# TigreGotico/phoonnx

Hardware: AMD Instinct MI355X
Metric: audio samples/sec (22.05 kHz), batch-32 256-phoneme utterances (higher is better)
Workload: dtype f32 (f16x3 split: fp32 operands as two fp16 planes, three MFMA products, fp32 accumulate)

## Files before the change

phoonnx_amd/build.py:

```python
import os
import shutil
import subprocess
import sys

HERE = os.path.dirname(os.path.abspath(__file__))
CSRC = os.path.join(HERE, "csrc")
LIB = os.path.join(HERE, "libvitsmi.so")
SOURCES = ["vitsmi.hip", "tu_conv_f32.hip", "tu_sx.hip", "tu_sx_s16.hip", "tu_sx_s16p.hip", "tu_sx_s32.hip", "tu_sx_bf16.hip", "tu_sx_h1.hip", "tu_pair.hip", "tu_pair16.hip", "g2p.hip",
           "model.cpp", "onnx_reader.cpp"]
HEADERS = sorted(f for f in os.listdir(CSRC) if f.endswith(".hpp")) + ["../../include/vitsmi.h", "../../include/g2pmi.h"]


def hipcc():
    for c in (os.environ.get("HIPCC"), shutil.which("hipcc"), "/opt/rocm/bin/hipcc"):
        if c and os.path.exists(c):
            return c
    raise RuntimeError("hipcc not found (ROCm toolchain required to build libvitsmi.so)")


def source_sha():
    import hashlib
    h = hashlib.sha256()
    for f in SOURCES + HEADERS:
        h.update(f.encode() + b"\0")
# ... 306 lines not shown
    objdir = os.path.join(HERE, "build")
    os.makedirs(objdir, exist_ok=True)
    base = [hipcc(), "--offload-arch=gfx950", "-O3", "-std=c++17", "-fPIC", "-Wno-unused-result",
            "-Rpass-analysis=kernel-resource-usage"]
    base[1:1] = os.environ.get("VITSMI_CXXFLAGS", "").split()

    isas = {}

    def compile_one(src):
        stem = os.path.splitext(src)[0]
        obj = os.path.join(objdir, stem + ".o")
        if not src.endswith(".hip"):
            r = subprocess.run(base + ["-x", "hip", "-c", os.path.join(CSRC, src), "-o", obj], capture_output=True, text=True)
            return src, obj, r
        tdir = os.path.join(objdir, "temps_" + stem)
        shutil.rmtree(tdir, ignore_errors=True)
        os.makedirs(tdir)
        tobj = os.path.join(tdir, stem + ".o")
        r = subprocess.run(base + ["-save-temps=obj", "-x", "hip", "-c", os.path.join(CSRC, src), "-o", tobj], capture_output=True, text=True)
        if r.returncode == 0:
            os.replace(tobj, obj)
            with open(os.path.join(tdir, stem + "-hip-amdgcn-amd-amdhsa-gfx950.s")) as f:
                isas[src] = f.read()
        shutil.rmtree(tdir, ignore_errors=True)
        return src, obj, r

    with ThreadPoolExecutor(max_workers=min(len(SOURCES), os.cpu_count() or 4)) as ex:
        results = list(ex.map(compile_one, SOURCES))
    spilled, spilled_src = {}, {}
    for src, _, r in results:
        if r.returncode != 0:
            sys.stderr.write(r.stdout + r.stderr)
            raise RuntimeError(f"hipcc failed compiling {src}")
        if verbose:
            sys.stderr.write(r.stderr)
        for k, v in spilling_kernels(r.stderr).items():
            spilled[k] = v
            spilled_src[k] = src
    no_spill = ("conv_sx_kernel", "conv_sx_pair16", "conv_sx_small_kernel", "attention_relpos16_kernel")
    bad = {k: v for k, v in spilled.items() if any(n in k for n in no_spill)}
    if bad:
        raise RuntimeError("kernels with asynchronous inline-asm loads must not spill registers: " + ", ".join(f"{k} ({v})" for k, v in bad.items()))
    hip_units = [u for u in SOURCES if u.endswith(".hip")]
    missing = [u for u in hip_units if u not in isas]
    if missing:
        raise RuntimeError(f"no device assembly was kept for {missing} (-save-temps=obj): the ISA checks cannot run")
# ... 40 lines not shown
```

phoonnx_amd/csrc/conv_engine.hip.hpp:

```cpp
#pragma once
#include <hip/hip_runtime.h>
#include <stdint.h>

#include <cstdio>

#include "sx_split.hip.hpp"

namespace vitsmi {

typedef float f32x16 __attribute__((ext_vector_type(16)));
typedef float f32x4 __attribute__((ext_vector_type(4)));
typedef float f32x2 __attribute__((ext_vector_type(2)));

enum : int {
    PRO_LRELU = 1,
    PRO_MASK = 2,
    EPI_RELU = 4,
    EPI_MASK = 8,
    EPI_RES = 16,
    EPI_ACC = 32,
    EPI_DIV = 64,
    EPI_COUPLING = 128,
    EPI_WN = 256,
    EPI_WN_FIRST = 512,
// ... 429 lines not shown
                for (int r = 0; r < 16; r++) v[r] = v[r] * mk_sel + ad[n % NB][r];
            } else {
#pragma unroll
                for (int r = 0; r < 16; r++) v[r] *= mk_sel;
            }
            if ((flags & EPI_RES) && (flags & EPI_ACC)) {
                float oo[16];
#pragma unroll
                for (int r = 0; r < 16; r++) oo[r] = orow_m[r] >= 0 ? ob[orow_m[r] + tt] : 0.f;
#pragma unroll
                for (int r = 0; r < 16; r++) v[r] += oo[r];
            }
            if (flags & EPI_DIV) {
#pragma unroll
                for (int r = 0; r < 16; r++) v[r] = v[r] / div;
            }
#pragma unroll
            for (int r = 0; r < 16; r++)
                if (orow_m[r] >= 0) obm[orow_m[r] + tt] = lrelu_f(v[r], oslope);
            if (planes_m) {
#pragma unroll
                for (int q = 0; q < 4; q++) {
                    unsigned wa[2], wb[2];
                    split2h_pair_pk(lrelu_f(v[4 * q], oslope), lrelu_f(v[4 * q + 1], oslope), wa[0], wa[1], pk);
                    split2h_pair_pk(lrelu_f(v[4 * q + 2], oslope), lrelu_f(v[4 * q + 3], oslope), wb[0], wb[1], pk);
                    const int64_t cell = ((int64_t)((mblk0 + m) * 4 + q) * T + t) * 8 + 4 * hi;
                    *reinterpret_cast<u32x2 *>(plb + cell) = u32x2{wa[0], wb[0]};
                    *reinterpret_cast<u32x2 *>(plb + plane_elems + cell) = u32x2{wa[1], wb[1]};
                }
            }
            if (ob2 && !is_wn) {
#pragma unroll
                for (int r = 0; r < 16; r++)
                    if (orow_m[r] >= 0) ob2[orow_m[r] + tt] = lrelu_f(v[r], oslope2);
            }
        }
    }
    if (a.peak) sx_publish_peak(a.peak, (int)(blockIdx.x + blockIdx.y + blockIdx.z), pk);
}

inline int conv_tile_m(int cfg) { return cfg == 2 ? 128 : ((cfg == 1 || cfg == 3) ? 64 : 32); }
inline int conv_tile_n(int cfg) {
    switch (cfg) {
        case 0: return 512;
        case 1: return 256;
        case 2: return 128;
        case 3: return 64;
        case 5: return 64;
// ... 75 lines not shown
```

phoonnx_amd/csrc/conv_sx_engine.hip.hpp:

```cpp
#pragma once
#include <hip/hip_runtime.h>
#include <stdint.h>

#include <cstdio>
#include <cstdlib>
#include <string>
#include <utility>

#include "conv_engine.hip.hpp"

#ifndef SX_CFG0_WIDE
#define SX_CFG0_WIDE 0
#endif
#ifndef SX16_SPREAD
#define SX16_SPREAD 0
#endif
#ifndef SX16_PRIO
#define SX16_PRIO 0
#endif
#ifndef SX16_ABL
#define SX16_ABL 0
#endif
#ifndef SX16_NA_SMALL
#define SX16_NA_SMALL 2
// ... 303 lines not shown
            xroff[it] = xrok[it] ? (uint32_t)(((int64_t)kh * T + t) * 32) : 0u;
        }
    }
    auto xload = [&](int chunk) {
        const float *cbase = xrb + (int64_t)(2 * chunk) * T * 8;
        static_for<NXC>([&](auto I) {
            constexpr int it = decltype(I)::value;
            if (it < nxc) {
                xst[it][0] = global_read128_x<0>(xroff[it], cbase);
                xst[it][1] = global_read128_x<16>(xroff[it], cbase);
            }
        });
    };
    auto xstore = [&](uint32_t xoff) {
        const float isl = a.islope;
        static_for<NXC>([&](auto I) {
            constexpr int it = decltype(I)::value;
            if (it < nxc) {
                int kh, col;
                xcell(it, kh, col);
                if (kh < 2) {
                    float v[8];
#pragma unroll
                    for (int e = 0; e < 8; e++) {
                        const float x = xrok[it] ? __uint_as_float(xst[it][e >> 2][e & 3]) : 0.f;
                        v[e] = fmaxf(x, x * isl);
                    }
                    u32x4 w0, w1, w2;
                    unsigned p0[4], p1[4], p2[4];
#pragma unroll
                    for (int e = 0; e < 4; e++) {
                        if constexpr (F16) split2h_pair_pk(v[2 * e], v[2 * e + 1], p0[e], p1[e], pk);
                        else split3_pair(v[2 * e], v[2 * e + 1], p0[e], p1[e], p2[e]);
                    }
                    w0 = u32x4{p0[0], p0[1], p0[2], p0[3]};
                    w1 = u32x4{p1[0], p1[1], p1[2], p1[3]};
                    const uint32_t ad = lds0 + xoff + (uint32_t)(kh * LW + col) * 16u;
                    const uint32_t pb = (uint32_t)(2 * LW) * 16u;
                    ds_write128(ad, w0);
                    if constexpr (NPL > 1) ds_write128(ad + pb, w1);
                    if constexpr (!F16 && NPL > 2) {
                        w2 = u32x4{p2[0], p2[1], p2[2], p2[3]};
                        ds_write128(ad + 2 * pb, w2);
                    }
                }
            }
        });
    };
    const int nxv = RAWIN ? 2 * nxc : (fastx ? nx_issued : nit);

// ... 606 lines not shown
        co0 = u == 1 ? row0 : (row0 / (32 * u)) * 32;
        t = t0 + (wn * NW + n) * 32 + l31;
    };
    auto cell_at = [&](int co0, int r, int t, int q) -> int64_t {
        return ((int64_t)((co0 >> 3) + q) * Tout + (t * u + r)) * 8 + 4 * hi;
    };
    auto issue_adds = [&](auto R, auto P) {
        constexpr int rr = decltype(R)::value, pp = decltype(P)::value;
        constexpr int m = rr / (NW / 2), n0 = (rr % (NW / 2)) * 2;
#pragma unroll
        for (int j = 0; j < 2; j++) {
            int co0, r, t;
            geom(m, n0 + j, co0, r, t);
            const int tl = t < T ? t : T - 1;
#pragma unroll
            for (int q = 0; q < 4; q++) {
                const int64_t c = cell_at(co0, r, tl, q);
                if (respl) {
                    if (res_epi) {
                        float o4[4];
                        if constexpr (H1) {
                            unact4h(*reinterpret_cast<const u32x2 *>(resplb + c), unsl, o4);
                        } else {
                            float h0[4], h1[4];
                            unact4h(*reinterpret_cast<const u32x2 *>(resplb + c), 1.f, h0);
                            unact4h(*reinterpret_cast<const u32x2 *>(resplb + plane_elems + c), 1.f, h1);
#pragma unroll
                            for (int e = 0; e < 4; e++) {
                                const float v = __builtin_fmaf(h1[e], 1.f / 2048.f, h0[e]);
                                o4[e] = v < 0.f ? v * unsl : v;
                            }
                        }
                        adb[pp][j][q] = f32x4{o4[0], o4[1], o4[2], o4[3]};
                    } else if (has_add)
                        adb[pp][j][q] = *reinterpret_cast<const f32x4 *>(rawb + c);
                } else if (has_add)
                    adb[pp][j][q] = *reinterpret_cast<const f32x4 *>(addp + c);
                if (two_adds) ad2[j][q] = *reinterpret_cast<const f32x4 *>(rawb + c);
            }
        }
    };
    if constexpr (PIPE) issue_adds(std::integral_constant<int, 0>{}, std::integral_constant<int, 0>{});
    static_for<NRND>([&](auto R) {
        constexpr int rr = decltype(R)::value;
        constexpr int m = rr / (NW / 2), n0 = (rr % (NW / 2)) * 2;
        constexpr int pp = PIPE ? (rr & 1) : 0;
        if constexpr (PIPE) {
            if constexpr (rr + 1 < NRND) issue_adds(std::integral_constant<int, rr + 1>{}, std::integral_constant<int, (rr + 1) & 1>{});
        } else
            issue_adds(R, std::integral_constant<int, 0>{});
        int co0m, rm, tm;
        geom(m, n0, co0m, rm, tm);
        const int row0 = mt * BM + (wm * MW + m) * 32;
        f32x4 bq[4];
// ... 18 lines not shown
#pragma unroll
                for (int e = 0; e < 4; e++) {
                    if constexpr (F16) v[e] = __builtin_fmaf(acc[m][n][4 * q + e], wsc, bq[q][e]);
                    else v[e] = acc[m][n][4 * q + e] + bq[q][e];
                }
                if constexpr (PRE) v += pre[rr][j][q];
                if (has_add) v += adb[pp][j][q];
                if (two_adds) v += ad2[j][q];
                if (flags & EPI_DIV) {
#pragma unroll
                    for (int e = 0; e < 4; e++) v[e] = v[e] / rdiv;
                }
                if (flags & SX_HAS_RAW) {
                    f32x4 o = v;
                    if (flags & SX_RAW_ACT) {
#pragma unroll
                        for (int e = 0; e < 4; e++) o[e] = fmaxf(v[e], v[e] * oslope);
                    }
                    *reinterpret_cast<f32x4 *>(rawb + cell) = o;
                }
                if (flags & SX_HAS_PL) {
                    f32x4 o = v;
                    if (flags & SX_PL_ACT) {
#pragma unroll
                        for (int e = 0; e < 4; e++) o[e] = fmaxf(v[e], v[e] * oslope2);
                    }
                    unsigned wa[3], wb[3];
                    if constexpr (H1) {
                        wa[0] = cvt1h_pair_pk(o[0], o[1], pk);
                        wb[0] = cvt1h_pair_pk(o[2], o[3], pk);
                    } else if constexpr (F16) {
                        split2h_pair_pk(o[0], o[1], wa[0], wa[1], pk);
                        split2h_pair_pk(o[2], o[3], wb[0], wb[1], pk);
                    } else {
                        split3_pair(o[0], o[1], wa[0], wa[1], wa[2]);
                        split3_pair(o[2], o[3], wb[0], wb[1], wb[2]);
                    }
#pragma unroll
                    for (int pl = 0; pl < NPL; pl++)
                        *reinterpret_cast<u32x2 *>(plb + pl * plane_elems + cell) = u32x2{wa[pl], wb[pl]};
                }
            }
        }
    });
    if constexpr (F16) {
        if (a.peak) {
            if constexpr (S16) sx_publish_peak_at(a.peak, (int)blockIdx.x, pk, reinterpret_cast<float *>(lds_sx));
            else sx_publish_peak(a.peak, (int)blockIdx.x, pk);
// ... 110 lines not shown
    if (rawin && (cfg == 0 || 2 * a.LW > 768 || !a.xr || (long long)a.T * 64 + 64 >= (1ll << 32))) return hipErrorInvalidValue;
    if (a.oslope == 0.f) a.oslope = 1.f;
    if (a.oslope2 == 0.f) a.oslope2 = 1.f;
    if (a.islope == 0.f) a.islope = 1.f;
    if (a.Cin % 16 || a.Cout % 32 || a.Cr % 32 || a.Cout % BM) return hipErrorInvalidValue;
    a.NT = (a.T + BN - 1) / BN;
    a.MT = a.Cout / BM;
    a.B = B;
    const long long nb = (long long)a.NT * B;
    if (nb == 0) return hipSuccess;
    a.xgs = a.NT >= (2 << sx_xcd_group_shift()) ? sx_xcd_group_shift() : 0;
    const long long per_round = 8ll << a.xgs;
    const long long wgs = (nb + per_round - 1) / per_round * per_round * a.MT;
    if (wgs >= (1ll << 31)) return hipErrorInvalidValue;
    dim3 grid((unsigned)wgs, 1, 1);
    int epi = a.flags & (EPI_RES | EPI_ACC | EPI_DIV);
    if (a.out_raw && !(a.flags & SX_NO_RAW_STORE)) epi |= SX_HAS_RAW | (a.oslope != 1.f ? SX_RAW_ACT : 0);
    if (a.out_pl && !(a.flags & SX_GATE)) epi |= SX_HAS_PL | (a.oslope2 != 1.f ? SX_PL_ACT : 0);
    if (a.bias_b) epi |= SX_HAS_BIASB;
    if (a.res_pl && nprod == 2 && (a.flags & EPI_RES)) {
        if (a.res || rawin || (a.flags & (SX_WN_RMW | SX_GATE))) return hipErrorInvalidValue;
        epi |= SX_RES_PL;
        if (a.res_unslope == 0.f) a.res_unslope = 1.f;
    }
    if (a.flags & SX_WN_RMW) {
        const bool p_acc = (a.flags & EPI_ACC) != 0;
        if (rawin || nprod != 2 || a.ups != 1 || (a.row_split < a.Cout && !a.out_raw2) ||
            (a.row_split && !a.out_raw && (p_acc || !a.out_pl)) || a.row_split % 32 || a.Cout % 32 || a.row_split > a.Cout ||
            a.pl_rows % 32 || a.pl_rows > (a.pl_of2 ? a.Cout - a.row_split : a.row_split) || (a.pl_rows && !a.out_pl) || a.bias_b ||
            (a.flags & SX_GATE) || ((a.flags & SX_PLANAR_COUPLING) && !p_acc) ||
            ((a.flags & EPI_RES) && (!a.res || p_acc)) || ((a.flags & EPI_MASK) && !a.len))
            return hipErrorInvalidValue;
        epi = -2;
    }
    if (a.flags & SX_GATE) {
        if (rawin || (cfg != 1 && cfg != 3) || (nprod != 2 && nprod != 6) || a.ups != 1 || (!a.out_raw && !a.out_pl) || (a.Cr & 63) ||
            lds < (size_t)2 * (sx_tile_n(cfg) / 64) * 4 * 1024)
            return hipErrorInvalidValue;
        epi |= SX_GATE | SX_HAS_RAW;
    }
    const bool early_ok = rawin && (nprod == 2 || (nprod == 6 && cfg == 2)) && (a.flags & EPI_RES) && !(a.flags & (DBG_NO_DMA | DBG_NO_EPI)) &&
                          a.res == a.xr && a.ups == 1 && a.out_raw && !(a.flags & SX_NO_RAW_STORE) && !a.out_pl && !a.bias_b &&
                          a.oslope == 1.f && (!(a.flags & EPI_DIV) || (a.flags & EPI_ACC));
    if (early_ok && epi != -2) epi |= SX_RES_EARLY;
    if (epi != -2) {
        if ((epi & EPI_RES) && !((nprod == 1 || (epi & SX_RES_PL)) ? (const void *)a.res_pl : (const void *)a.res)) return hipErrorInvalidValue;
// ... 187 lines not shown
```

phoonnx_amd/csrc/conv_sx_pair.hip.hpp:

```cpp
#pragma once
#include <cstdlib>
#include "conv_sx_engine.hip.hpp"

namespace vitsmi {

struct SxPairArgs {
    const float *xr;
    float islope, mslope;
    int T;
    const u32x4 *wp1, *wp2;
    const float *bias1, *bias2;
    float wscale1, wscale2;
    float *out_raw;
    const float *zeros;
    int C, nchunks;
    int K1, dil1, pad1;
    int K2, dil2, pad2;
    int LW1;
    unsigned x_bytes;
    int LW2;
    unsigned y_chunk_bytes;
    int BNo, NT, B;
    int flags;
    float div;
// ... 8 lines not shown
    int nchain;
    unsigned a_ring;
    unsigned bias_off;
    unsigned long long *prof;
    SxRagged rag;
    int xgs = 0;
};

#ifndef SX_PAIR_PROF
#define SX_PAIR_PROF 0
#endif
#ifndef SX_PAIR_SHARED_A
#define SX_PAIR_SHARED_A 0
#endif
#ifndef SX_PAIR_ALIAS
#define SX_PAIR_ALIAS 0
#endif
#ifndef SX_PAIR_DEPTH32
#define SX_PAIR_DEPTH32 2
#endif
#ifndef SX_PAIR_DEPTH64
#define SX_PAIR_DEPTH64 2
#endif
#ifndef SX_PAIR_EARLY_ACC
#define SX_PAIR_EARLY_ACC 0
#endif
#ifndef SX_PAIR_WGS32
#define SX_PAIR_WGS32 3
#endif
#ifndef SX_PAIR_EARLY32
#define SX_PAIR_EARLY32 1
#endif
#ifndef SX_PAIR_ST_SC1
#define SX_PAIR_ST_SC1 0
#endif
#ifndef SX_PAIR_ONE_READ64
#define SX_PAIR_ONE_READ64 1
#endif
#ifndef SX_PAIR_ONE_READ32
#define SX_PAIR_ONE_READ32 1
#endif
template <int MW, int NW, int WM, int WN, int EPI, bool CHAIN, int NCH = 1>
__global__ __launch_bounds__(256, (NW == 2 && !SX_PAIR_EARLY_ACC && NCH == 1) ? SX_PAIR_WGS32 : 2) void conv_sx_pair_kernel(SxPairArgs a) {
    constexpr int BN = NW * WN * 32, NH = NW / 2;
    static_assert(NCH == 1 || (CHAIN && NW == 2 && (EPI & EPI_ACC) == 0), "fused chains: 32 channels, no external running sum");
    constexpr bool ONE_READ = NW == 4 ? SX_PAIR_ONE_READ64 != 0 : SX_PAIR_ONE_READ32 != 0;
    constexpr bool EARLY = ONE_READ || (NW == 2 && SX_PAIR_EARLY32);
    constexpr int DEPTH = NW == 2 ? SX_PAIR_DEPTH32 : SX_PAIR_DEPTH64;
    static_assert(DEPTH >= 2 && DEPTH <= 6, "wait_a covers up to five younger sets");
    constexpr bool ACC = (EPI & EPI_ACC) != 0 && SX_PAIR_EARLY_ACC;
    static_assert(!(ONE_READ && ACC), "the running sum is not pulled into the single-read prologue");
    static_assert(WM * WN == 4 && MW == 1 && BN == 256, "one block row per wave, 256 columns");
    constexpr int NPW = 2, STEPBYTES = WM * MW * NPW * 1024;
    constexpr int MAXCH = WM * 2;
    extern __shared__ __attribute__((aligned(16))) unsigned char lds_sx[];
    const int tid = threadIdx.x, lane = tid & 63;
    const int wave = __builtin_amdgcn_readfirstlane(tid >> 6);
    const int wm = wave / WN, wn = wave % WN;
    const int l31 = lane & 31, hi = lane >> 5;
    const int wg_xcd = blockIdx.x & 7, wg_seq = blockIdx.x >> 3;
    const int tile_nb = __builtin_amdgcn_readfirstlane(sx_xcd_tile(wg_seq, wg_xcd, a.xgs));
    if (tile_nb >= a.NT * a.B) return;
    const int b = tile_nb / a.NT, t0 = (tile_nb - b * a.NT) * a.BNo;
    const int t1 = t0 - a.pad2;
    const int T = a.T, LW = a.LW1;
    const int TV = __builtin_amdgcn_readfirstlane(sx_valid_cols(a.rag, b, T));
    if (t0 >= TV) return;
    const uint32_t lds0 = (uint32_t)(uintptr_t)lds_sx;
    const uint32_t XB = a.x_bytes;
    const char *wbase1 = reinterpret_cast<const char *>(a.wp1) + wm * (MW * NPW * 1024);
    const char *wbase2 = reinterpret_cast<const char *>(a.wp2) + wm * (MW * NPW * 1024);
    const float *xrb = a.xr + (int64_t)b * a.C * T;
    float pk = 0.f;

    struct ASet {
        u32x4 fa[2];
    };
    const uint32_t voff0 = (uint32_t)lane * 16u;
    auto load_a = [&](ASet &f, const char *wb, int step) {
        const char *sb = wb + (int64_t)step * STEPBYTES;
        f.fa[0] = global_read128<0>(voff0, sb);
        f.fa[1] = global_read128<1024>(voff0, sb);
    };

    f32x4 pre[NW / 2][2][4], ad[EARLY && ACC ? NW / 2 : 1][2][4];
    auto load_res = [&](const float *base, f32x4 (*dst)[2][4]) {
        static_for<NW / 2>([&](auto R) {
            constexpr int rr = decltype(R)::value;
#pragma unroll
            for (int j = 0; j < 2; j++) {
                const int row0 = wm * 32;
                const int t = t1 + (wn * NW + rr * 2 + j) * 32 + l31;
                const int tl = t < 0 ? 0 : (t < T ? t : T - 1);
#pragma unroll
                for (int q = 0; q < 4; q++) {
                    const float *p = base + ((int64_t)((row0 >> 3) + q) * T + tl) * 8 + 4 * hi;
                    if constexpr (EARLY) dst[rr][j][q] = __builtin_bit_cast(f32x4, global_read128_v<0>(p));
                    else dst[rr][j][q] = *reinterpret_cast<const f32x4 *>(p);
                }
            }
        });
    };
    auto load_pre = [&]() { load_res(xrb, pre); };

#if SX_PAIR_PROF
    auto stamp = [&]() {
        unsigned long long t;
        __builtin_amdgcn_sched_barrier(0);
        asm volatile("s_memtime %0\n\ts_waitcnt lgkmcnt(0)" : "=s"(t)::"memory");
        __builtin_amdgcn_sched_barrier(0);
        return t;
    };
    unsigned long long tp[8];
    tp[0] = stamp();
#endif
    if constexpr (NW == 2 && WM == 1 && NCH == 1 && SX_PAIR_SHARED_A != 0)
        for (int g = 0; g < 3; g++)
            if (g < ((a.nchunks * a.K1) >> 1)) {
                const int sub = wave >> 1, pl = wave & 1;
                lds_dma<16>(wbase1 + (int64_t)(2 * g + sub) * STEPBYTES + pl * 1024 + lane * 16,
                            reinterpret_cast<float *>(lds_sx + a.a_ring + (unsigned)((g * 2 + sub) * 2048 + pl * 1024)));
            }
    constexpr bool BIAS_LDS = NCH == 1;
    if constexpr (BIAS_LDS) {
        if (wave == 0) {
            constexpr int CC = WM * 32;
            const int k = lane - (lane >= CC / 4 ? CC / 4 : 0);
            const float *bp = lane < CC / 4 ? a.bias1 : a.bias2;
            const void *src = (bp && lane < CC / 2) ? static_cast<const void *>(bp + 4 * k) : static_cast<const void *>(a.zeros + 4 * (lane & 31));
            lds_dma<16>(src, reinterpret_cast<float *>(lds_sx + a.bias_off));
        }
    }
    auto bias_from_lds = [&](int conv, f32x4 (&bq)[4]) __attribute__((always_inline)) {
        u32x4 t4[4];
#pragma unroll
        for (int q = 0; q < 4; q++)
            asm volatile("ds_read_b128 %0, %1" : "=v"(t4[q]) : "v"(lds0 + a.bias_off + (uint32_t)(conv * (WM * 32) + wm * 32 + 8 * q + 4 * hi) * 4u) : "memory");
        asm volatile("s_waitcnt lgkmcnt(0)" ::: "memory");
        __builtin_amdgcn_sched_barrier(0);
#pragma unroll
        for (int q = 0; q < 4; q++) bq[q] = __builtin_bit_cast(f32x4, t4[q]);
    };
    constexpr int NXC = 3;
    if constexpr (ONE_READ) {
        constexpr int NXH = MAXCH, NG = 2 * MAXCH;
        const int HW = LW - 256, pad1 = a.pad1;
        const int nhc = HW * NG, nxh = (nhc + 255) >> 8;
        u32x4 hst[NXH][2];
        bool hin[NXH], hok[NXH];
        uint32_t hlds[NXH];
        const float *hp[NXH];
#pragma unroll
        for (int it = 0; it < NXH; it++) {
            const int h = it * 256 + tid;
            hin[it] = h < nhc;
            const int g = hin[it] ? h / HW : 0;
            const int c = hin[it] ? h - g * HW : 0;
            const int col = c < pad1 ? c : c + 256;
            const int t = t1 - pad1 + col;
            hok[it] = hin[it] && t >= 0 && t < TV;
            hp[it] = xrb + (hok[it] ? ((int64_t)g * T + t) * 8 : (int64_t)0);
            hlds[it] = lds0 + (uint32_t)(g >> 1) * XB + (uint32_t)((g & 1) * LW + col) * 16u;
        }
        static_for<NXH>([&](auto I) {
            constexpr int it = decltype(I)::value;
            if (it < nxh) {
                hst[it][0] = global_read128_v<0>(hp[it]);
                hst[it][1] = global_read128_v<16>(hp[it]);
            }
        });
        load_pre();
        const float isl = a.islope;
        static_for<NW>([&](auto N) {
            constexpr int n = decltype(N)::value;
            asm volatile("s_waitcnt vmcnt(%0)" ::"n"(4 * (NW - 1 - n)) : "memory");
            __builtin_amdgcn_sched_barrier(0);
#if SX_PAIR_PROF
            if constexpr (n == 0) tp[1] = stamp();
#endif
            if constexpr (n == 0) {
                static_for<NXH>([&](auto I) {
                    constexpr int it = decltype(I)::value;
                    if (it < nxh && hin[it]) {
                        float v[8];
#pragma unroll
                        for (int e = 0; e < 8; e++) {
                            const float x = hok[it] ? __uint_as_float(hst[it][e >> 2][e & 3]) : 0.f;
                            v[e] = fmaxf(x, x * isl);
                        }
                        unsigned p0[4], p1[4];
#pragma unroll
                        for (int e = 0; e < 4; e++) split2h_pair_pk(v[2 * e], v[2 * e + 1], p0[e], p1[e], pk);
                        ds_write128(hlds[it], u32x4{p0[0], p0[1], p0[2], p0[3]});
                        ds_write128(hlds[it] + (uint32_t)(2 * LW) * 16u, u32x4{p1[0], p1[1], p1[2], p1[3]});
                    }
                });
            }
            const int col = (wn * NW + n) * 32 + l31;
            const int t = t1 + col;
            const bool ok = t >= 0 && t < TV;
#pragma unroll
            for (int q = 0; q < 4; q++) {
                float v[4];
#pragma unroll
                for (int e = 0; e < 4; e++) {
                    const float x = ok ? pre[n / 2][n % 2][q][e] : 0.f;
                    v[e] = fmaxf(x, x * isl);
                }
                unsigned wa[2], wb[2];
                split2h_pair_pk(v[0], v[1], wa[0], wa[1], pk);
                split2h_pair_pk(v[2], v[3], wb[0], wb[1], pk);
                const int g = 4 * wm + q;
                const uint32_t cell = lds0 + (uint32_t)(g >> 1) * XB + (uint32_t)((g & 1) * LW + pad1 + col) * 16u + 8u * hi;
                asm volatile("ds_write_b64 %0, %1" ::"v"(cell), "v"(u32x2{wa[0], wb[0]}) : "memory");
                asm volatile("ds_write_b64 %0, %1" ::"v"(cell + (uint32_t)(2 * LW) * 16u), "v"(u32x2{wa[1], wb[1]}) : "memory");
            }
            asm volatile("" : "+v"(pk));
        });
    } else {
        u32x4 xst[MAXCH][NXC][2];
        const int nxc = (2 * LW + 255) >> 8;
        uint32_t xroff[NXC];
        bool xrok[NXC];
        int xkh[NXC], xcol[NXC];
#pragma unroll
        for (int it = 0; it < NXC; it++) {
            const int i = it * 256 + tid;
            const int kh = (i >= LW ? 1 : 0) + (i >= 2 * LW ? 1 : 0);
            const int col = i - kh * LW;
            const int t = t1 - a.pad1 + col;
            xkh[it] = kh;
            xcol[it] = col;
            xrok[it] = it < nxc && kh < 2 && t >= 0 && t < TV;
            xroff[it] = xrok[it] ? (uint32_t)(((int64_t)kh * T + t) * 32) : 0u;
        }
        static_for<MAXCH>([&](auto CH) {
            constexpr int ch = decltype(CH)::value;
            const float *cbase = xrb + (int64_t)(2 * ch) * T * 8;
            static_for<NXC>([&](auto I) {
                constexpr int it = decltype(I)::value;
                if (it < nxc) {
                    xst[ch][it][0] = global_read128_x<0>(xroff[it], cbase);
                    xst[ch][it][1] = global_read128_x<16>(xroff[it], cbase);
                }
            });
        });
        if constexpr (EARLY) {
            load_pre();
            if constexpr (ACC) {
                load_res(a.out_raw + (int64_t)b * a.C * T, ad);
                asm volatile("s_waitcnt vmcnt(16)" ::: "memory");
            } else
                asm volatile("s_waitcnt vmcnt(8)" ::: "memory");
        } else
            asm volatile("s_waitcnt vmcnt(0)" ::: "memory");
#if SX_PAIR_PROF
        tp[1] = stamp();
#endif
        const float isl = a.islope;
        static_for<MAXCH>([&](auto CH) {
            constexpr int ch = decltype(CH)::value;
            static_for<NXC>([&](auto I) {
                constexpr int it = decltype(I)::value;
                if (it < nxc && xkh[it] < 2) {
                    float v[8];
#pragma unroll
                    for (int e = 0; e < 8; e++) {
                        const float x = xrok[it] ? __uint_as_float(xst[ch][it][e >> 2][e & 3]) : 0.f;
                        v[e] = fmaxf(x, x * isl);
                    }
                    unsigned p0[4], p1[4];
#pragma unroll
                    for (int e = 0; e < 4; e++) split2h_pair_pk(v[2 * e], v[2 * e + 1], p0[e], p1[e], pk);
                    const uint32_t ad = lds0 + (uint32_t)ch * XB + (uint32_t)(xkh[it] * LW + xcol[it]) * 16u;
                    ds_write128(ad, u32x4{p0[0], p0[1], p0[2], p0[3]});
                    ds_write128(ad + (uint32_t)(2 * LW) * 16u, u32x4{p1[0], p1[1], p1[2], p1[3]});
                }
            });
        });
    }

    f32x16 acc[NW];
    auto zero_acc = [&]() {
#pragma unroll
        for (int n = 0; n < NW; n++)
#pragma unroll
            for (int r = 0; r < 16; r++) acc[n][r] = 0.f;
    };
    zero_acc();
    u32x4 fb[NW][2];
    auto load_b_half = [&](auto H, uint32_t rows, uint32_t pstride) {
        constexpr int h = decltype(H)::value;
        static_for<NH>([&](auto N) {
            constexpr int n = h * NH + decltype(N)::value;
            fb[n][0] = ds_read128<n * 512>(rows);
            fb[n][1] = ds_read128<n * 512>(rows + pstride);
        });
    };
    auto mma_half = [&](const ASet &f, auto H) {
        constexpr int h = decltype(H)::value;
#pragma unroll
// ... 156 lines not shown
            step(fa1, fa0, 2 * g + 1, true);
        }
    };

    struct ChainPar {
        const char *wb1, *wb2;
        const float *bias1, *bias2;
        float ws1, ws2;
        int K1, dil1, K2, dil2;
        uint32_t xoff, yoff;
    };
    auto chain_par = [&](int ci) {
        ChainPar c;
        if constexpr (NCH == 1) {
            c = ChainPar{wbase1, wbase2, a.bias1, a.bias2, a.wscale1, a.wscale2, a.K1, a.dil1, a.K2, a.dil2, 0u, 0u};
        } else {
            const auto &h = a.ch[ci];
            c = ChainPar{reinterpret_cast<const char *>(h.wp1) + wm * (MW * NPW * 1024),
                         reinterpret_cast<const char *>(h.wp2) + wm * (MW * NPW * 1024),
                         h.bias1, h.bias2, h.wscale1, h.wscale2, h.K1, h.dil1, h.K2, h.dil2, (uint32_t)h.xoff, (uint32_t)h.yoff};
        }
        return c;
    };
    static_assert(NCH == 1 || EARLY, "fused chains keep x in registers from the prologue on");
    const uint32_t ylds = NCH > 1 ? lds0 + (uint32_t)a.nchunks * XB : lds0;
    f32x4 xkeep[NCH > 1 ? NW / 2 : 1][2][4], tot[NCH > 1 ? NW / 2 : 1][2][4];
#if SX_PAIR_ALIAS
    ASet f1s[DEPTH + 1];
    ASet(&f2s)[DEPTH + 1] = f1s;
#else
    ASet f1s[DEPTH + 1], f2s[DEPTH + 1];
#endif
#pragma unroll 1
    for (int ci = 0; ci < NCH; ci++) {
    const ChainPar cp = chain_par(ci);
    if constexpr (NCH > 1) {
        if (ci > 0) {
#pragma unroll
            for (int rr = 0; rr < NW / 2; rr++)
#pragma unroll
                for (int j = 0; j < 2; j++)
#pragma unroll
                    for (int q = 0; q < 4; q++) pre[rr][j][q] = xkeep[rr][j][q];
            zero_acc();
        }
    }
    if constexpr (!SHA) load_a(f1s[0], cp.wb1, 0);
    if (ci == 0) {
        asm volatile("s_waitcnt lgkmcnt(0)" ::: "memory");
#if SX_PAIR_PROF
        tp[2] = stamp();
#endif
        __builtin_amdgcn_s_barrier();
#if SX_PAIR_PROF
        tp[3] = stamp();
#endif
    }
    __builtin_amdgcn_sched_barrier(0);
    if constexpr (SHA)
        run_conv_sha(f1s[0], f1s[1], cp.wb1, cp.K1, cp.dil1, lds0 + (uint32_t)(hi * LW + wn * (NW * 32) + l31 + (int)cp.xoff) * 16u,
                     XB, (uint32_t)(2 * LW) * 16u);
    else
        run_conv(f1s, cp.wb1, cp.K1, cp.dil1, lds0 + (uint32_t)(hi * LW + wn * (NW * 32) + l31 + (int)cp.xoff) * 16u, XB,
                 (uint32_t)(2 * LW) * 16u);

#if SX_PAIR_PROF
    tp[4] = stamp();
#endif
    if constexpr (CHAIN && !EARLY) load_pre();

    if constexpr (!SHA) load_a(f2s[0], cp.wb2, 0);
    asm volatile("s_waitcnt lgkmcnt(0)" ::: "memory");
    __builtin_amdgcn_s_barrier();
    __builtin_amdgcn_sched_barrier(0);
    if constexpr (SHA) sha_prefetch(cp.wb2, cp.K2);
    {
        const float wsc = cp.ws1, msl = a.mslope;
        const float *biasp = cp.bias1 ? cp.bias1 : a.zeros;
        const int b_on = cp.bias1 ? 1 : 0;
        const uint32_t YC = a.y_chunk_bytes, LW2 = (uint32_t)a.LW2;
        const int row0 = wm * 32;
        f32x4 bq[4];
        if constexpr (BIAS_LDS) bias_from_lds(0, bq);
        else {
#pragma unroll
            for (int q = 0; q < 4; q++) bq[q] = *reinterpret_cast<const f32x4 *>(biasp + (row0 + 8 * q + 4 * hi) * b_on);
        }
#pragma unroll
        for (int n = 0; n < NW; n++) {
            const int col = (wn * NW + n) * 32 + l31;
            const int t = t1 + col;
            const bool live = t >= 0 && t < TV;
#pragma unroll
            for (int q = 0; q < 4; q++) {
                float o[4];
#pragma unroll
                for (int e = 0; e < 4; e++) {
                    float v = __builtin_fmaf(acc[n][4 * q + e], wsc, bq[q][e]);
                    if constexpr (CHAIN) {
                        if constexpr (NCH > 1) {
                            if (ci == 0) xkeep[n / 2][n % 2][q][e] = pre[n / 2][n % 2][q][e];
                        }
                        v += pre[n / 2][n % 2][q][e];
                        pre[n / 2][n % 2][q][e] = v;
                    }
                    o[e] = live ? fmaxf(v, v * msl) : 0.f;
                }
                unsigned wa[2], wb[2];
                split2h_pair_pk(o[0], o[1], wa[0], wa[1], pk);
                split2h_pair_pk(o[2], o[3], wb[0], wb[1], pk);
                const int g = 4 * wm + q;
                const uint32_t cell = ylds + (uint32_t)(g >> 1) * YC + ((uint32_t)(g & 1) * LW2 + (uint32_t)(col + a.pad2)) * 16u + 8u * hi;
                asm volatile("ds_write_b64 %0, %1" ::"v"(cell), "v"(u32x2{wa[0], wb[0]}) : "memory");
                asm volatile("ds_write_b64 %0, %1" ::"v"(cell + 2u * LW2 * 16u), "v"(u32x2{wa[1], wb[1]}) : "memory");
            }
            asm volatile("" : "+v"(pk));
        }
    }
    zero_acc();
    asm volatile("s_waitcnt lgkmcnt(0)" ::: "memory");
    __builtin_amdgcn_s_barrier();
    __builtin_amdgcn_sched_barrier(0);
#if SX_PAIR_PROF
    tp[5] = stamp();
#endif

    if constexpr (SHA)
        run_conv_sha(f2s[0], f2s[1], cp.wb2, cp.K2, cp.dil2, ylds + (uint32_t)(hi * a.LW2 + wn * (NW * 32) + l31 + (int)cp.yoff) * 16u,
                     a.y_chunk_bytes, (uint32_t)(2 * a.LW2) * 16u);
    else
        run_conv(f2s, cp.wb2, cp.K2, cp.dil2, ylds + (uint32_t)(hi * a.LW2 + wn * (NW * 32) + l31 + (int)cp.yoff) * 16u,
                 a.y_chunk_bytes, (uint32_t)(2 * a.LW2) * 16u);
#if SX_PAIR_PROF
    tp[6] = stamp();
#endif
    if constexpr (!CHAIN && !EARLY) load_pre();

    {
        constexpr int flags = EPI;
        float *rawb = a.out_raw + (int64_t)b * a.C * T;
        const float wsc = cp.ws2, rdiv = a.div;
        const float *biasp = cp.bias2 ? cp.bias2 : a.zeros;
        const int b_on = cp.bias2 ? 1 : 0;
        const int row0 = wm * 32;
        f32x4 bq[4];
        if constexpr (BIAS_LDS) bias_from_lds(1, bq);
        else {
#pragma unroll
            for (int q = 0; q < 4; q++) bq[q] = *reinterpret_cast<const f32x4 *>(biasp + (row0 + 8 * q + 4 * hi) * b_on);
        }
        static_for<NW / 2>([&](auto R) {
            constexpr int rr = decltype(R)::value;
            f32x4 adl[2][4];
            if constexpr ((flags & EPI_ACC) != 0 && !(EARLY && ACC)) {
#pragma unroll
                for (int j = 0; j < 2; j++) {
                    const int t = t1 + (wn * NW + rr * 2 + j) * 32 + l31;
                    const int tl = t < 0 ? 0 : (t < T ? t : T - 1);
#pragma unroll
                    for (int q = 0; q < 4; q++)
                        adl[j][q] = *reinterpret_cast<const f32x4 *>(rawb + ((int64_t)((row0 >> 3) + q) * T + tl) * 8 + 4 * hi);
                }
            }
#pragma unroll
            for (int j = 0; j < 2; j++) {
                const int n = rr * 2 + j;
                const int col = (wn * NW + n) * 32 + l31;
                const int t = t1 + col;
                const bool kept = !(col < a.pad2 || col >= a.pad2 + a.BNo || t >= TV);
                if constexpr (NCH == 1) {
                    if (!kept) continue;
                }
#pragma unroll
                for (int q = 0; q < 4; q++) {
                    f32x4 v;
#pragma unroll
                    for (int e = 0; e < 4; e++) v[e] = __builtin_fmaf(acc[n][4 * q + e], wsc, bq[q][e]);
                    v += pre[rr][j][q];
                    if constexpr (NCH > 1) {
                        if (ci > 0) v += tot[rr][j][q];
                        tot[rr][j][q] = v;
                        if (ci < NCH - 1 || !kept) continue;
                    }
                    if constexpr ((flags & EPI_ACC) != 0) {
                        if constexpr (EARLY && ACC) v += ad[rr][j][q];
                        else v += adl[j][q];
                    }
                    if constexpr ((flags & EPI_DIV) != 0) {
#pragma unroll
                        for (int e = 0; e < 4; e++) v[e] = v[e] / rdiv;
                    }
#if SX_PAIR_ST_SC1
                    {
                        float *sp = rawb + ((int64_t)((row0 >> 3) + q) * T + t) * 8 + 4 * hi;
                        const f32x4 sv = v;
                        asm volatile("global_store_dwordx4 %0, %1, off sc1" ::"v"(sp), "v"(sv) : "memory");
                    }
#else
                    *reinterpret_cast<f32x4 *>(rawb + ((int64_t)((row0 >> 3) + q) * T + t) * 8 + 4 * hi) = v;
#endif
                }
            }
        });
    }
    }
#if SX_PAIR_PROF
    asm volatile("s_waitcnt vmcnt(0)" ::: "memory");
    tp[7] = stamp();
    if (a.prof && tid == 0) {
// ... 167 lines not shown
```

phoonnx_amd/csrc/sx_split.hip.hpp:

```cpp
#pragma once
#include <hip/hip_runtime.h>
#include <stdint.h>

#include <atomic>

namespace vitsmi {

typedef float sxf32x2 __attribute__((ext_vector_type(2)));
typedef _Float16 f16x2 __attribute__((ext_vector_type(2)));
typedef unsigned u32x4 __attribute__((ext_vector_type(4)));
typedef unsigned u32x2 __attribute__((ext_vector_type(2)));

constexpr int kSxPeakSlots = 64;
constexpr float kF16Max = 65504.f;

inline thread_local bool g_launch_name_on = false;
inline thread_local char g_launch_name[128];

__device__ __forceinline__ unsigned cvt_pk_f16(float lo, float hi) {
    const sxf32x2 v = {lo, hi};
    return __builtin_bit_cast(unsigned, __builtin_convertvector(v, f16x2));
}
__device__ __forceinline__ void split2h_pair(float x, float y, unsigned &w0, unsigned &w1) {
    x = __builtin_amdgcn_fmed3f(x, -65504.f, 65504.f);
    y = __builtin_amdgcn_fmed3f(y, -65504.f, 65504.f);
    w0 = cvt_pk_f16(x, y);
    const f16x2 h = __builtin_bit_cast(f16x2, w0);
    w1 = cvt_pk_f16((x - (float)h[0]) * 2048.f, (y - (float)h[1]) * 2048.f);
}
__device__ __forceinline__ void split2h_pair_pk(float x, float y, unsigned &w0, unsigned &w1, float &pk) {
    pk = __builtin_fmaxf(pk, __builtin_fmaxf(__builtin_fabsf(x), __builtin_fabsf(y)));
    split2h_pair(x, y, w0, w1);
}
__device__ __forceinline__ unsigned cvt1h_pair_pk(float x, float y, float &pk) {
    pk = __builtin_fmaxf(pk, __builtin_fmaxf(__builtin_fabsf(x), __builtin_fabsf(y)));
    return cvt_pk_f16(__builtin_amdgcn_fmed3f(x, -65504.f, 65504.f), __builtin_amdgcn_fmed3f(y, -65504.f, 65504.f));
}
__device__ __forceinline__ void unact4h(u32x2 w, float unslope, float (&o)[4]) {
    const unsigned wx = w.x, wy = w.y;
    const f16x2 a = __builtin_bit_cast(f16x2, wx), b = __builtin_bit_cast(f16x2, wy);
    const float v[4] = {(float)a[0], (float)a[1], (float)b[0], (float)b[1]};
#pragma unroll
    for (int e = 0; e < 4; e++) o[e] = v[e] < 0.f ? v[e] * unslope : v[e];
}

constexpr int kSxPeakStride = 32;
constexpr int kSxMaxDynLds = 160 * 1024 - 256;
inline hipError_t sx_allow_big_lds(const void *kern, std::atomic<uint64_t> &done) {
    int dev = 0;
    if (hipGetDevice(&dev) != hipSuccess) return hipGetLastError();
    const uint64_t bit = 1ull << (dev & 63);
    if (done.load(std::memory_order_acquire) & bit) return hipSuccess;
    const hipError_t e = hipFuncSetAttribute(kern, hipFuncAttributeMaxDynamicSharedMemorySize, kSxMaxDynLds);
    if (e == hipSuccess) done.fetch_or(bit, std::memory_order_release);
    return e;
}
__device__ __forceinline__ void sx_publish_peak_at(unsigned *slots, int slot_idx, float pk, float *s_pk) {
#pragma unroll
    for (int o = 32; o > 0; o >>= 1) pk = __builtin_fmaxf(pk, __shfl_xor(pk, o, 64));
    __syncthreads();
    if ((threadIdx.x & 63) == 0) s_pk[threadIdx.x >> 6] = pk;
    __syncthreads();
    if (threadIdx.x == 0) {
        pk = __builtin_fmaxf(__builtin_fmaxf(s_pk[0], s_pk[1]), __builtin_fmaxf(s_pk[2], s_pk[3]));
        unsigned *slot = slots + (slot_idx & (kSxPeakSlots - 1)) * kSxPeakStride;
        const unsigned bits = __float_as_uint(pk);
// ... 35 lines not shown
```

Measured before the change: 145.2 million.

## Use packed and mixed-precision ALU ops in split/unsplit and lrelu epilogues; drop legacy pair prologue

Rewrites the fp16 two-plane split to build the residual plane with v_fma_mix instructions, fuses the peak tracking into v_max3, and adds packed-f32 leaky-ReLU, FMA and unsplit helpers used across the sx and pair conv kernels. The pair kernel's non-single-read prologue and early-accumulate variants are removed, and LDS writes now use immediate offsets computed per unrolled column. The aim is fewer VALU instructions in the prologue and epilogue of the conv kernels. The new split rounds slightly differently from the old path, and the unsplit now relies on res_unslope >= 1, which is enforced by a new argument check.

```diff
diff --git a/phoonnx_amd/build.py b/phoonnx_amd/build.py
--- a/phoonnx_amd/build.py
+++ b/phoonnx_amd/build.py
@@ -352,6 +352,11 @@
             os.replace(tobj, obj)
             with open(os.path.join(tdir, stem + "-hip-amdgcn-amd-amdhsa-gfx950.s")) as f:
                 isas[src] = f.read()
+            keep = os.environ.get("VITSMI_KEEP_ISA")
+            if keep:
+                os.makedirs(keep, exist_ok=True)
+                with open(os.path.join(keep, stem + ".s"), "w") as f:
+                    f.write(isas[src])
         shutil.rmtree(tdir, ignore_errors=True)
         return src, obj, r
 
diff --git a/phoonnx_amd/csrc/conv_engine.hip.hpp b/phoonnx_amd/csrc/conv_engine.hip.hpp
--- a/phoonnx_amd/csrc/conv_engine.hip.hpp
+++ b/phoonnx_amd/csrc/conv_engine.hip.hpp
@@ -475,8 +475,8 @@
 #pragma unroll
                 for (int q = 0; q < 4; q++) {
                     unsigned wa[2], wb[2];
-                    split2h_pair_pk(lrelu_f(v[4 * q], oslope), lrelu_f(v[4 * q + 1], oslope), wa[0], wa[1], pk);
-                    split2h_pair_pk(lrelu_f(v[4 * q + 2], oslope), lrelu_f(v[4 * q + 3], oslope), wb[0], wb[1], pk);
+                    split2h_pair_pk_c(lrelu_f(v[4 * q], oslope), lrelu_f(v[4 * q + 1], oslope), wa[0], wa[1], pk);
+                    split2h_pair_pk_c(lrelu_f(v[4 * q + 2], oslope), lrelu_f(v[4 * q + 3], oslope), wb[0], wb[1], pk);
                     const int64_t cell = ((int64_t)((mblk0 + m) * 4 + q) * T + t) * 8 + 4 * hi;
                     *reinterpret_cast<u32x2 *>(plb + cell) = u32x2{wa[0], wb[0]};
                     *reinterpret_cast<u32x2 *>(plb + plane_elems + cell) = u32x2{wa[1], wb[1]};
diff --git a/phoonnx_amd/csrc/conv_sx_engine.hip.hpp b/phoonnx_amd/csrc/conv_sx_engine.hip.hpp
--- a/phoonnx_amd/csrc/conv_sx_engine.hip.hpp
+++ b/phoonnx_amd/csrc/conv_sx_engine.hip.hpp
@@ -349,10 +349,9 @@
                 if (kh < 2) {
                     float v[8];
 #pragma unroll
-                    for (int e = 0; e < 8; e++) {
-                        const float x = xrok[it] ? __uint_as_float(xst[it][e >> 2][e & 3]) : 0.f;
-                        v[e] = fmaxf(x, x * isl);
-                    }
+                    for (int e = 0; e < 8; e++) v[e] = xrok[it] ? __uint_as_float(xst[it][e >> 2][e & 3]) : 0.f;
+#pragma unroll
+                    for (int e = 0; e < 4; e++) lrelu_pair(v[2 * e], v[2 * e + 1], isl);
                     u32x4 w0, w1, w2;
                     unsigned p0[4], p1[4], p2[4];
 #pragma unroll
@@ -1005,14 +1004,8 @@
                         if constexpr (H1) {
                             unact4h(*reinterpret_cast<const u32x2 *>(resplb + c), unsl, o4);
                         } else {
-                            float h0[4], h1[4];
-                            unact4h(*reinterpret_cast<const u32x2 *>(resplb + c), 1.f, h0);
-                            unact4h(*reinterpret_cast<const u32x2 *>(resplb + plane_elems + c), 1.f, h1);
-#pragma unroll
-                            for (int e = 0; e < 4; e++) {
-                                const float v = __builtin_fmaf(h1[e], 1.f / 2048.f, h0[e]);
-                                o4[e] = v < 0.f ? v * unsl : v;
-                            }
+                            unsplit4h(*reinterpret_cast<const u32x2 *>(resplb + c),
+                                      *reinterpret_cast<const u32x2 *>(resplb + plane_elems + c), unsl, o4);
                         }
                         adb[pp][j][q] = f32x4{o4[0], o4[1], o4[2], o4[3]};
                     } else if (has_add)
@@ -1077,8 +1070,15 @@
                 if (flags & SX_HAS_PL) {
                     f32x4 o = v;
                     if (flags & SX_PL_ACT) {
-#pragma unroll
-                        for (int e = 0; e < 4; e++) o[e] = fmaxf(v[e], v[e] * oslope2);
+                        if constexpr (F16 && !H1) {
+                            float l[4] = {v[0], v[1], v[2], v[3]};
+                            lrelu_pair(l[0], l[1], oslope2);
+                            lrelu_pair(l[2], l[3], oslope2);
+                            o = f32x4{l[0], l[1], l[2], l[3]};
+                        } else {
+#pragma unroll
+                            for (int e = 0; e < 4; e++) o[e] = fmaxf(v[e], v[e] * oslope2);
+                        }
                     }
                     unsigned wa[3], wb[3];
                     if constexpr (H1) {
@@ -1235,6 +1235,7 @@
         if (a.res || rawin || (a.flags & (SX_WN_RMW | SX_GATE))) return hipErrorInvalidValue;
         epi |= SX_RES_PL;
         if (a.res_unslope == 0.f) a.res_unslope = 1.f;
+        if (!(a.res_unslope >= 1.f)) return hipErrorInvalidValue;
     }
     if (a.flags & SX_WN_RMW) {
         const bool p_acc = (a.flags & EPI_ACC) != 0;
diff --git a/phoonnx_amd/csrc/conv_sx_pair.hip.hpp b/phoonnx_amd/csrc/conv_sx_pair.hip.hpp
--- a/phoonnx_amd/csrc/conv_sx_pair.hip.hpp
+++ b/phoonnx_amd/csrc/conv_sx_pair.hip.hpp
@@ -54,34 +54,18 @@
 #ifndef SX_PAIR_DEPTH64
 #define SX_PAIR_DEPTH64 2
 #endif
-#ifndef SX_PAIR_EARLY_ACC
-#define SX_PAIR_EARLY_ACC 0
-#endif
 #ifndef SX_PAIR_WGS32
 #define SX_PAIR_WGS32 3
 #endif
-#ifndef SX_PAIR_EARLY32
-#define SX_PAIR_EARLY32 1
-#endif
 #ifndef SX_PAIR_ST_SC1
 #define SX_PAIR_ST_SC1 0
 #endif
-#ifndef SX_PAIR_ONE_READ64
-#define SX_PAIR_ONE_READ64 1
-#endif
-#ifndef SX_PAIR_ONE_READ32
-#define SX_PAIR_ONE_READ32 1
-#endif
 template <int MW, int NW, int WM, int WN, int EPI, bool CHAIN, int NCH = 1>
-__global__ __launch_bounds__(256, (NW == 2 && !SX_PAIR_EARLY_ACC && NCH == 1) ? SX_PAIR_WGS32 : 2) void conv_sx_pair_kernel(SxPairArgs a) {
+__global__ __launch_bounds__(256, (NW == 2 && NCH == 1) ? SX_PAIR_WGS32 : 2) void conv_sx_pair_kernel(SxPairArgs a) {
     constexpr int BN = NW * WN * 32, NH = NW / 2;
     static_assert(NCH == 1 || (CHAIN && NW == 2 && (EPI & EPI_ACC) == 0), "fused chains: 32 channels, no external running sum");
-    constexpr bool ONE_READ = NW == 4 ? SX_PAIR_ONE_READ64 != 0 : SX_PAIR_ONE_READ32 != 0;
-    constexpr bool EARLY = ONE_READ || (NW == 2 && SX_PAIR_EARLY32);
     constexpr int DEPTH = NW == 2 ? SX_PAIR_DEPTH32 : SX_PAIR_DEPTH64;
     static_assert(DEPTH >= 2 && DEPTH <= 6, "wait_a covers up to five younger sets");
-    constexpr bool ACC = (EPI & EPI_ACC) != 0 && SX_PAIR_EARLY_ACC;
-    static_assert(!(ONE_READ && ACC), "the running sum is not pulled into the single-read prologue");
     static_assert(WM * WN == 4 && MW == 1 && BN == 256, "one block row per wave, 256 columns");
     constexpr int NPW = 2, STEPBYTES = WM * MW * NPW * 1024;
     constexpr int MAXCH = WM * 2;
@@ -115,7 +99,7 @@
         f.fa[1] = global_read128<1024>(voff0, sb);
     };
 
-    f32x4 pre[NW / 2][2][4], ad[EARLY && ACC ? NW / 2 : 1][2][4];
+    f32x4 pre[NW / 2][2][4];
     auto load_res = [&](const float *base, f32x4 (*dst)[2][4]) {
         static_for<NW / 2>([&](auto R) {
             constexpr int rr = decltype(R)::value;
@@ -127,8 +111,7 @@
 #pragma unroll
                 for (int q = 0; q < 4; q++) {
                     const float *p = base + ((int64_t)((row0 >> 3) + q) * T + tl) * 8 + 4 * hi;
-                    if constexpr (EARLY) dst[rr][j][q] = __builtin_bit_cast(f32x4, global_read128_v<0>(p));
-                    else dst[rr][j][q] = *reinterpret_cast<const f32x4 *>(p);
+                    dst[rr][j][q] = __builtin_bit_cast(f32x4, global_read128_v<0>(p));
                 }
             }
         });
@@ -173,8 +156,7 @@
 #pragma unroll
         for (int q = 0; q < 4; q++) bq[q] = __builtin_bit_cast(f32x4, t4[q]);
     };
-    constexpr int NXC = 3;
-    if constexpr (ONE_READ) {
+    {
         constexpr int NXH = MAXCH, NG = 2 * MAXCH;
         const int HW = LW - 256, pad1 = a.pad1;
         const int nhc = HW * NG, nxh = (nhc + 255) >> 8;
@@ -216,10 +198,9 @@
                     if (it < nxh && hin[it]) {
                         float v[8];
 #pragma unroll
-                        for (int e = 0; e < 8; e++) {
-                            const float x = hok[it] ? __uint_as_float(hst[it][e >> 2][e & 3]) : 0.f;
-                            v[e] = fmaxf(x, x * isl);
-                        }
+                        for (int e = 0; e < 8; e++) v[e] = hok[it] ? __uint_as_float(hst[it][e >> 2][e & 3]) : 0.f;
+#pragma unroll
+                        for (int e = 0; e < 4; e++) lrelu_pair(v[2 * e], v[2 * e + 1], isl);
                         unsigned p0[4], p1[4];
 #pragma unroll
                         for (int e = 0; e < 4; e++) split2h_pair_pk(v[2 * e], v[2 * e + 1], p0[e], p1[e], pk);
@@ -235,80 +216,18 @@
             for (int q = 0; q < 4; q++) {
                 float v[4];
 #pragma unroll
-                for (int e = 0; e < 4; e++) {
-                    const float x = ok ? pre[n / 2][n % 2][q][e] : 0.f;
-                    v[e] = fmaxf(x, x * isl);
-                }
+                for (int e = 0; e < 4; e++) v[e] = ok ? pre[n / 2][n % 2][q][e] : 0.f;
+                lrelu_pair(v[0], v[1], isl);
+                lrelu_pair(v[2], v[3], isl);
                 unsigned wa[2], wb[2];
                 split2h_pair_pk(v[0], v[1], wa[0], wa[1], pk);
                 split2h_pair_pk(v[2], v[3], wb[0], wb[1], pk);
                 const int g = 4 * wm + q;
-                const uint32_t cell = lds0 + (uint32_t)(g >> 1) * XB + (uint32_t)((g & 1) * LW + pad1 + col) * 16u + 8u * hi;
-                asm volatile("ds_write_b64 %0, %1" ::"v"(cell), "v"(u32x2{wa[0], wb[0]}) : "memory");
-                asm volatile("ds_write_b64 %0, %1" ::"v"(cell + (uint32_t)(2 * LW) * 16u), "v"(u32x2{wa[1], wb[1]}) : "memory");
+                const uint32_t cell = lds0 + (uint32_t)(g >> 1) * XB + (uint32_t)((g & 1) * LW + pad1 + wn * (NW * 32) + l31) * 16u + 8u * hi;
+                asm volatile("ds_write_b64 %0, %1 offset:%2" ::"v"(cell), "v"(u32x2{wa[0], wb[0]}), "n"(n * 512) : "memory");
+                asm volatile("ds_write_b64 %0, %1 offset:%2" ::"v"(cell + (uint32_t)(2 * LW) * 16u), "v"(u32x2{wa[1], wb[1]}), "n"(n * 512) : "memory");
             }
             asm volatile("" : "+v"(pk));
-        });
-    } else {
-        u32x4 xst[MAXCH][NXC][2];
-        const int nxc = (2 * LW + 255) >> 8;
-        uint32_t xroff[NXC];
-        bool xrok[NXC];
-        int xkh[NXC], xcol[NXC];
-#pragma unroll
-        for (int it = 0; it < NXC; it++) {
-            const int i = it * 256 + tid;
-            const int kh = (i >= LW ? 1 : 0) + (i >= 2 * LW ? 1 : 0);
-            const int col = i - kh * LW;
-            const int t = t1 - a.pad1 + col;
-            xkh[it] = kh;
-            xcol[it] = col;
-            xrok[it] = it < nxc && kh < 2 && t >= 0 && t < TV;
-            xroff[it] = xrok[it] ? (uint32_t)(((int64_t)kh * T + t) * 32) : 0u;
-        }
-        static_for<MAXCH>([&](auto CH) {
-            constexpr int ch = decltype(CH)::value;
-            const float *cbase = xrb + (int64_t)(2 * ch) * T * 8;
-            static_for<NXC>([&](auto I) {
-                constexpr int it = decltype(I)::value;
-                if (it < nxc) {
-                    xst[ch][it][0] = global_read128_x<0>(xroff[it], cbase);
-                    xst[ch][it][1] = global_read128_x<16>(xroff[it], cbase);
-                }
-            });
-        });
-        if constexpr (EARLY) {
-            load_pre();
-            if constexpr (ACC) {
-                load_res(a.out_raw + (int64_t)b * a.C * T, ad);
-                asm volatile("s_waitcnt vmcnt(16)" ::: "memory");
-            } else
-                asm volatile("s_waitcnt vmcnt(8)" ::: "memory");
-        } else
-            asm volatile("s_waitcnt vmcnt(0)" ::: "memory");
-#if SX_PAIR_PROF
-        tp[1] = stamp();
-#endif
-        const float isl = a.islope;
-        static_for<MAXCH>([&](auto CH) {
-            constexpr int ch = decltype(CH)::value;
-            static_for<NXC>([&](auto I) {
-                constexpr int it = decltype(I)::value;
-                if (it < nxc && xkh[it] < 2) {
-                    float v[8];
-#pragma unroll
-                    for (int e = 0; e < 8; e++) {
-                        const float x = xrok[it] ? __uint_as_float(xst[ch][it][e >> 2][e & 3]) : 0.f;
-                        v[e] = fmaxf(x, x * isl);
-                    }
-                    unsigned p0[4], p1[4];
-#pragma unroll
-                    for (int e = 0; e < 4; e++) split2h_pair_pk(v[2 * e], v[2 * e + 1], p0[e], p1[e], pk);
-                    const uint32_t ad = lds0 + (uint32_t)ch * XB + (uint32_t)(xkh[it] * LW + xcol[it]) * 16u;
-                    ds_write128(ad, u32x4{p0[0], p0[1], p0[2], p0[3]});
-                    ds_write128(ad + (uint32_t)(2 * LW) * 16u, u32x4{p1[0], p1[1], p1[2], p1[3]});
-                }
-            });
         });
     }
 
@@ -511,7 +430,6 @@
         }
         return c;
     };
-    static_assert(NCH == 1 || EARLY, "fused chains keep x in registers from the prologue on");
     const uint32_t ylds = NCH > 1 ? lds0 + (uint32_t)a.nchunks * XB : lds0;
     f32x4 xkeep[NCH > 1 ? NW / 2 : 1][2][4], tot[NCH > 1 ? NW / 2 : 1][2][4];
 #if SX_PAIR_ALIAS
@@ -556,7 +474,6 @@
 #if SX_PAIR_PROF
     tp[4] = stamp();
 #endif
-    if constexpr (CHAIN && !EARLY) load_pre();
 
     if constexpr (!SHA) load_a(f2s[0], cp.wb2, 0);
     asm volatile("s_waitcnt lgkmcnt(0)" ::: "memory");
@@ -575,8 +492,8 @@
 #pragma unroll
             for (int q = 0; q < 4; q++) bq[q] = *reinterpret_cast<const f32x4 *>(biasp + (row0 + 8 * q + 4 * hi) * b_on);
         }
-#pragma unroll
-        for (int n = 0; n < NW; n++) {
+        static_for<NW>([&](auto N) {
+            constexpr int n = decltype(N)::value;
             const int col = (wn * NW + n) * 32 + l31;
             const int t = t1 + col;
             const bool live = t >= 0 && t < TV;
@@ -584,27 +501,36 @@
             for (int q = 0; q < 4; q++) {
                 float o[4];
 #pragma unroll
-                for (int e = 0; e < 4; e++) {
-                    float v = __builtin_fmaf(acc[n][4 * q + e], wsc, bq[q][e]);
+                for (int e = 0; e < 4; e += 2) {
+                    sxf32x2 v = fma_pair(acc[n][4 * q + e], acc[n][4 * q + e + 1], wsc, bq[q][e], bq[q][e + 1]);
                     if constexpr (CHAIN) {
                         if constexpr (NCH > 1) {
-                            if (ci == 0) xkeep[n / 2][n % 2][q][e] = pre[n / 2][n % 2][q][e];
+                            if (ci == 0) {
+                                xkeep[n / 2][n % 2][q][e] = pre[n / 2][n % 2][q][e];
+                                xkeep[n / 2][n % 2][q][e + 1] = pre[n / 2][n % 2][q][e + 1];
+                            }
                         }
-                        v += pre[n / 2][n % 2][q][e];
-                        pre[n / 2][n % 2][q][e] = v;
+                        v += sxf32x2{pre[n / 2][n % 2][q][e], pre[n / 2][n % 2][q][e + 1]};
+                        pre[n / 2][n % 2][q][e] = v[0];
+                        pre[n / 2][n % 2][q][e + 1] = v[1];
                     }
-                    o[e] = live ? fmaxf(v, v * msl) : 0.f;
+                    o[e] = v[0];
+                    o[e + 1] = v[1];
                 }
+                lrelu_pair(o[0], o[1], msl);
+                lrelu_pair(o[2], o[3], msl);
+#pragma unroll
+                for (int e = 0; e < 4; e++) o[e] = live ? o[e] : 0.f;
                 unsigned wa[2], wb[2];
                 split2h_pair_pk(o[0], o[1], wa[0], wa[1], pk);
                 split2h_pair_pk(o[2], o[3], wb[0], wb[1], pk);
                 const int g = 4 * wm + q;
-                const uint32_t cell = ylds + (uint32_t)(g >> 1) * YC + ((uint32_t)(g & 1) * LW2 + (uint32_t)(col + a.pad2)) * 16u + 8u * hi;
-                asm volatile("ds_write_b64 %0, %1" ::"v"(cell), "v"(u32x2{wa[0], wb[0]}) : "memory");
-                asm volatile("ds_write_b64 %0, %1" ::"v"(cell + 2u * LW2 * 16u), "v"(u32x2{wa[1], wb[1]}) : "memory");
+                const uint32_t cell = ylds + (uint32_t)(g >> 1) * YC + ((uint32_t)(g & 1) * LW2 + (uint32_t)(wn * (NW * 32) + l31 + a.pad2)) * 16u + 8u * hi;
+                asm volatile("ds_write_b64 %0, %1 offset:%2" ::"v"(cell), "v"(u32x2{wa[0], wb[0]}), "n"(n * 512) : "memory");
+                asm volatile("ds_write_b64 %0, %1 offset:%2" ::"v"(cell + 2u * LW2 * 16u), "v"(u32x2{wa[1], wb[1]}), "n"(n * 512) : "memory");
             }
             asm volatile("" : "+v"(pk));
-        }
+        });
     }
     zero_acc();
     asm volatile("s_waitcnt lgkmcnt(0)" ::: "memory");
@@ -623,7 +549,6 @@
 #if SX_PAIR_PROF
     tp[6] = stamp();
 #endif
-    if constexpr (!CHAIN && !EARLY) load_pre();
 
     {
         constexpr int flags = EPI;
@@ -641,7 +566,7 @@
         static_for<NW / 2>([&](auto R) {
             constexpr int rr = decltype(R)::value;
             f32x4 adl[2][4];
-            if constexpr ((flags & EPI_ACC) != 0 && !(EARLY && ACC)) {
+            if constexpr ((flags & EPI_ACC) != 0) {
 #pragma unroll
                 for (int j = 0; j < 2; j++) {
                     const int t = t1 + (wn * NW + rr * 2 + j) * 32 + l31;
@@ -672,8 +597,7 @@
                         if (ci < NCH - 1 || !kept) continue;
                     }
                     if constexpr ((flags & EPI_ACC) != 0) {
-                        if constexpr (EARLY && ACC) v += ad[rr][j][q];
-                        else v += adl[j][q];
+                        v += adl[j][q];
                     }
                     if constexpr ((flags & EPI_DIV) != 0) {
 #pragma unroll
diff --git a/phoonnx_amd/csrc/sx_split.hip.hpp b/phoonnx_amd/csrc/sx_split.hip.hpp
--- a/phoonnx_amd/csrc/sx_split.hip.hpp
+++ b/phoonnx_amd/csrc/sx_split.hip.hpp
@@ -25,12 +25,40 @@
     x = __builtin_amdgcn_fmed3f(x, -65504.f, 65504.f);
     y = __builtin_amdgcn_fmed3f(y, -65504.f, 65504.f);
     w0 = cvt_pk_f16(x, y);
+    const sxf32x2 s = sxf32x2{x, y} * 2048.f;
+    const float m = -2048.f;
+    asm("v_fma_mixlo_f16 %0, %1, %2, %3 op_sel:[0,0,0] op_sel_hi:[1,0,0]" : "=v"(w1) : "v"(w0), "s"(m), "v"(s[0]));
+    asm("v_fma_mixhi_f16 %0, %1, %2, %3 op_sel:[1,0,0] op_sel_hi:[1,0,0]" : "+v"(w1) : "v"(w0), "s"(m), "v"(s[1]));
+}
+__device__ __forceinline__ void split2h_pair_pk_c(float x, float y, unsigned &w0, unsigned &w1, float &pk) {
+    pk = __builtin_fmaxf(pk, __builtin_fmaxf(__builtin_fabsf(x), __builtin_fabsf(y)));
+    x = __builtin_amdgcn_fmed3f(x, -65504.f, 65504.f);
+    y = __builtin_amdgcn_fmed3f(y, -65504.f, 65504.f);
+    w0 = cvt_pk_f16(x, y);
     const f16x2 h = __builtin_bit_cast(f16x2, w0);
     w1 = cvt_pk_f16((x - (float)h[0]) * 2048.f, (y - (float)h[1]) * 2048.f);
 }
 __device__ __forceinline__ void split2h_pair_pk(float x, float y, unsigned &w0, unsigned &w1, float &pk) {
-    pk = __builtin_fmaxf(pk, __builtin_fmaxf(__builtin_fabsf(x), __builtin_fabsf(y)));
+    asm("v_max3_f32 %0, %0, |%1|, |%2|" : "+v"(pk) : "v"(x), "v"(y));
     split2h_pair(x, y, w0, w1);
+}
+__device__ __forceinline__ float max_nc(float a, float b) {
+    float r;
+    asm("v_max_f32 %0, %1, %2" : "=v"(r) : "v"(a), "v"(b));
+    return r;
+}
+__device__ __forceinline__ float min_nc(float a, float b) {
+    float r;
+    asm("v_min_f32 %0, %1, %2" : "=v"(r) : "v"(a), "v"(b));
+    return r;
+}
+__device__ __forceinline__ void lrelu_pair(float &x, float &y, float slope) {
+    const sxf32x2 m = sxf32x2{x, y} * slope;
+    x = max_nc(x, m[0]);
+    y = max_nc(y, m[1]);
+}
+__device__ __forceinline__ sxf32x2 fma_pair(float a0, float a1, float s, float b0, float b1) {
+    return __builtin_elementwise_fma(sxf32x2{a0, a1}, sxf32x2{s, s}, sxf32x2{b0, b1});
 }
 __device__ __forceinline__ unsigned cvt1h_pair_pk(float x, float y, float &pk) {
     pk = __builtin_fmaxf(pk, __builtin_fmaxf(__builtin_fabsf(x), __builtin_fabsf(y)));
@@ -42,6 +70,20 @@
     const float v[4] = {(float)a[0], (float)a[1], (float)b[0], (float)b[1]};
 #pragma unroll
     for (int e = 0; e < 4; e++) o[e] = v[e] < 0.f ? v[e] * unslope : v[e];
+}
+__device__ __forceinline__ void unsplit4h(u32x2 w0, u32x2 w1, float unslope, float (&o)[4]) {
+    const unsigned ax = w0.x, ay = w0.y, bx = w1.x, by = w1.y;
+    const float c = 1.f / 2048.f;
+    float v[4];
+    asm("v_fma_mix_f32 %0, %1, %2, %3 op_sel:[0,0,0] op_sel_hi:[1,0,1]" : "=v"(v[0]) : "v"(bx), "s"(c), "v"(ax));
+    asm("v_fma_mix_f32 %0, %1, %2, %3 op_sel:[1,0,1] op_sel_hi:[1,0,1]" : "=v"(v[1]) : "v"(bx), "s"(c), "v"(ax));
+    asm("v_fma_mix_f32 %0, %1, %2, %3 op_sel:[0,0,0] op_sel_hi:[1,0,1]" : "=v"(v[2]) : "v"(by), "s"(c), "v"(ay));
+    asm("v_fma_mix_f32 %0, %1, %2, %3 op_sel:[1,0,1] op_sel_hi:[1,0,1]" : "=v"(v[3]) : "v"(by), "s"(c), "v"(ay));
+    const sxf32x2 m0 = sxf32x2{v[0], v[1]} * unslope, m1 = sxf32x2{v[2], v[3]} * unslope;
+    o[0] = min_nc(v[0], m0[0]);
+    o[1] = min_nc(v[1], m0[1]);
+    o[2] = min_nc(v[2], m1[0]);
+    o[3] = min_nc(v[3], m1[1]);
 }
 
 constexpr int kSxPeakStride = 32;
```

Result: no change. 145.7 million, median of 6 (+0.3%).
